# AlexandreRouma/SDRPlusPlus

Measured on NVIDIA H100. Metric: complex IQ MSamples/s through FFT + 8-VFO WFM chain, higher is better.
Workload: dtype f32

## Files before the change

### sdrplusplus_b200/csrc/engine.cpp

```cpp
#include "engine.h"
#include <chrono>
#include "../../include/b200dsp.h"
#include <cmath>
#include <cstdarg>
#include <cstdio>
#include <cstring>
#include <algorithm>
#include <map>
#include <functional>
#include <cstdlib>

namespace b200 {

static thread_local char g_err[512] = "";
void set_error(const char* fmt, ...) {
    va_list ap;
    va_start(ap, fmt);
    vsnprintf(g_err, sizeof(g_err), fmt, ap);
    va_end(ap);
}
const char* last_error() { return g_err; }
int cuda_fail(cudaError_t e, const char* what) {
    set_error("CUDA error %d (%s) in %s", (int)e, cudaGetErrorString(e), what);
    if (e == cudaErrorNoDevice || e == cudaErrorInsufficientDriver) { return B200_ENODEV; }
    return B200_ECUDA;
}

struct TraceRec { const char* label; cudaEvent_t ev; };
static std::vector<TraceRec> g_trace;
static int g_trace_on = -1;
bool trace_on() {
    if (g_trace_on < 0) { const char* e = getenv("B200_TRACE"); g_trace_on = (e && *e && *e != '0') ? 1 : 0; }
    return g_trace_on == 1;
}
void trace_mark(const char* label, cudaStream_t s) {
// ... 112 lines not shown
    }
    taps_dirty = false;
    return 0;
}

int XdStage::plan(int n) {
    n_in = n;
    chunk_offset = offset;
    chunk_phase0 = phase;
    chunk_retuned = retuned && n > 0;
    chunk_w_prev = w_prev;
    if (n > 0) { retuned = false; }
    n_out = (offset < n) ? (n - offset + D - 1) / D : 0;
    offset = offset + n_out * D - n;
    phase += w * (unsigned long long)(long long)n;
    return n_out;
}

int FirCStage::configure(const std::vector<float>& t, int decim_) {
    ntaps = (int)t.size();
    decim = decim_;
    hist = ntaps - 1;
    htaps = t;
    int rc = taps.alloc((size_t)ntaps * sizeof(float));
    if (rc) { return rc; }
    B200_CK(cudaMemcpy(taps.p, t.data(), (size_t)ntaps * sizeof(float), cudaMemcpyHostToDevice));
    return upload_pm(t, decim, 1);
}
int FirCStage::plan(int n) {
    n_in = n;
    chunk_offset = offset;
    n_out = (offset < n) ? (n - offset + decim - 1) / decim : 0;
    offset = offset + n_out * decim - n;
    return n_out;
}

int PolyStage::configure(int interp_, int decim_, const std::vector<float>& t) {
    interp = interp_;
    decim = decim_;
    std::vector<float> b = build_polyphase_bank(interp, t, tpp);
    hist = tpp - 1;
    int rc = bank.alloc(b.size() * sizeof(float));
    if (rc) { return rc; }
    B200_CK(cudaMemcpy(bank.p, b.data(), b.size() * sizeof(float), cudaMemcpyHostToDevice));
    {
        std::vector<float> kl(((size_t)tpp * interp + 3) & ~(size_t)3, 0.0f);
        for (int ph = 0; ph < interp; ph++) {
            for (int k = 0; k < tpp; k++) { kl[(size_t)k * interp + ph] = b[(size_t)ph * tpp + k]; }
        }
        if ((rc = bank_kl.alloc(kl.size() * sizeof(float)))) { return rc; }
        B200_CK(cudaMemcpy(bank_kl.p, kl.data(), kl.size() * sizeof(float), cudaMemcpyHostToDevice));
    }
    return upload_pm(b, decim, interp);
}
int PolyStage::plan(int n) {
    n_in = n;
    chunk_phase = phase;
    chunk_offset = offset;
    long long avail = ((long long)n - offset) * interp - phase;
    long long no = avail > 0 ? (avail + decim - 1) / decim : 0;
    n_out = (int)no;
    long long tend = (long long)phase + no * decim;
    offset = (int)((long long)offset + tend / interp - n);
    phase = (int)(tend % interp);
    return n_out;
}
// ... 87 lines not shown
    B200_CK(cudaMemcpy(state.p, init_state, sizeof(init_state), cudaMemcpyHostToDevice));
    return 0;
}

int SeqStage::configure_noise_blanker(double rate, double level) {
    memset(&proto, 0, sizeof(proto));
    proto.kind = 3;
    proto.nb_rate = (float)rate;
    proto.nb_inv_rate = 1.0f - proto.nb_rate;
    proto.nb_level = (float)level;
    in_es = 2;
    out_es = 2;
    memset(init_state, 0, sizeof(init_state));
    init_state[7] = 1.0f;
    int rc = state.alloc(sizeof(init_state));
    if (rc) { return rc; }
    B200_CK(cudaMemcpy(state.p, init_state, sizeof(init_state), cudaMemcpyHostToDevice));
    return 0;
}
int FmIfStage::configure(int nbins) {
    if (!fmif_supported(nbins)) { set_error("FM IF noise reduction: %d bins (supported: 2 ... %d)", nbins, 64); return B200_EINVAL; }
    bins = nbins;
    hist = bins - 1;
    const std::vector<float> w = fmif_window(bins), t = dft_twiddles(bins);
    int rc;
    if ((rc = win.alloc(w.size() * sizeof(float), false)) || (rc = tw.alloc(t.size() * sizeof(float), false))) { return rc; }
    B200_CK(cudaMemcpy(win.p, w.data(), w.size() * sizeof(float), cudaMemcpyHostToDevice));
    B200_CK(cudaMemcpy(tw.p, t.data(), t.size() * sizeof(float), cudaMemcpyHostToDevice));
    return 0;
}

int Chain::finalize(int max_in, bool dbl_first, const FuseCfg* fuse) {
    if (st.empty()) { set_error("empty chain"); return B200_EINVAL; }
    int cap = max_in;
    if (dbl_first && st.size() >= 2 && st[0]->kind == K_XD) { st[1]->dbl = true; }
    for (auto& s : st) {
        if (s->kind != K_XD) {
            int rc = s->alloc_in(cap);
            if (rc) { return rc; }
        }
        else { s->cap_in = cap; }
        cap = s->max_out(cap);
    }
    {
        int c2 = max_in;
        for (auto& s : st) {
            if (s->kind == K_STEREO) {
                StereoStage* q = (StereoStage*)s.get();
                int rc2;
                if ((rc2 = q->p.alloc(((size_t)c2 + 8) * sizeof(float2), false)) || (rc2 = q->vco.alloc(((size_t)c2 + 8) * sizeof(float2), false))) { return rc2; }
            }
            c2 = s->max_out(c2);
        }
    }
    out_es = st.back()->out_es;
    out_cap = cap;
    int rc = out.alloc(((size_t)cap + 8) * out_es * sizeof(float));
    if (rc) { return rc; }
    if (fuse) { fcfg = *fuse; }
    rc = plan_fused();
    if (rc) { return rc; }
    B200_CK(cudaDeviceSynchronize());
    return 0;
}

static bool ft_fusable(const Stage* s) {
    switch (s->kind) {
    case K_FIRC: return s->in_es == 2;
    case K_POLY: return s->in_es == 2 && ((const PolyStage*)s)->interp <= 64;
    case K_QUAD: case K_FIRR: case K_M2S: return true;
    default: return false;
    }
}
static void ft_describe(const Stage* s, FtStage& d) {
    memset(&d, 0, sizeof(d));
    d.D = 1; d.L = 1; d.T = 1;
    d.hist = s->hist;
    d.es = s->in_es;
    switch (s->kind) {
    case K_FIRC: { const FirCStage* f = (const FirCStage*)s; d.kind = FT_FIRC; d.T = f->ntaps; d.D = f->decim; break; }
    case K_POLY: { const PolyStage* f = (const PolyStage*)s; d.kind = FT_POLY; d.T = f->tpp; d.D = f->decim; d.L = f->interp; break; }
    case K_QUAD: { const QuadStage* f = (const QuadStage*)s; d.kind = FT_QUAD; d.scale = f->inv_dev; break; }
    case K_FIRR: { const FirRStage* f = (const FirRStage*)s; d.kind = FT_FIRR; d.T = f->ntaps; d.dup = f->stereo; break; }
    default: d.kind = FT_M2S; d.dup = 1; break;
    }
    d.taps = s->taps_pm.as<float>();
    d.ntap_f = s->pm_floats;
}
static long long ft_need_len(const FtStage& d, long long len) {
    switch (d.kind) {
    case FT_FIRC: case FT_FIRR: return (len - 1) * d.D + d.T;
    case FT_POLY: return ((len - 1) * d.D + d.L - 1) / d.L + d.T + 1;
    case FT_QUAD: return len + 1;
// ... 363 lines not shown
        t.ev.push_back(a);
        t.ev.push_back(b);
    }
    cudaEvent_t t0 = t.ev[t.used], t1 = t.ev[t.used + 1];
    t.used += 2;
    cudaEventRecord(t0, s);
    return t1;
}
int Scheduler::group_stats(int group, double* ms_total, int* n) {
    if (group < 0 || group > 2) { set_error("bad timer group"); return B200_EINVAL; }
    Timer& t = timers[group];
    double tot = 0.0;
    for (size_t i = 0; i + 1 < t.used; i += 2) {
        B200_CK(cudaEventSynchronize(t.ev[i + 1]));
        float ms = 0.0f;
        B200_CK(cudaEventElapsedTime(&ms, t.ev[i], t.ev[i + 1]));
        tot += ms;
    }
    *ms_total = tot;
    *n = (int)(t.used / 2);
    t.used = 0;
    return 0;
}
int Scheduler::reset_raw() {
    if (raw_hist.p) { B200_CK(cudaMemset(raw_hist.p, 0, raw_hist.bytes)); B200_CK(cudaDeviceSynchronize()); }
    return 0;
}

static int apply_pending_taps(FirCStage* f, cudaStream_t s) {
    if (f->pending.empty()) { return 0; }
    (void)s;
    B200_CK(cudaDeviceSynchronize());
    const int newT = (int)f->pending.size(), oldT = f->ntaps;
    const int newH = newT - 1, oldH = oldT - 1;
    const size_t bytes = ((size_t)newH + f->cap_in + Scheduler::STAGE_SPARE) * f->in_es * sizeof(float);
    DevBuf nb, nb2;
    int rc = nb.alloc(bytes);
    if (rc) { return rc; }
    if (f->dbl && (rc = nb2.alloc(bytes))) { return rc; }
    int keep = std::min(newH, oldH);
    const float* live = f->dbl ? ((f->par ? f->inbuf.as<float>() : f->inbuf_alt.as<float>())) : f->inbuf.as<float>();
    float* live_new = f->dbl ? ((f->par ? nb.as<float>() : nb2.as<float>())) : nb.as<float>();
    if (keep > 0) {
        B200_CK(cudaMemcpy(live_new + (size_t)(newH - keep) * f->in_es, live + (size_t)(oldH - keep) * f->in_es,
                           (size_t)keep * f->in_es * sizeof(float), cudaMemcpyDeviceToDevice));
    }
    std::swap(f->inbuf.p, nb.p);
    std::swap(f->inbuf.bytes, nb.bytes);
    if (f->dbl) {
        std::swap(f->inbuf_alt.p, nb2.p);
        std::swap(f->inbuf_alt.bytes, nb2.bytes);
    }
    if (f->fmid) {
        DevBuf h0, h1;
        const size_t hb = ((size_t)newH + 8) * f->in_es * sizeof(float);
        if ((rc = h0.alloc(hb)) || (rc = h1.alloc(hb))) { return rc; }
        if (keep > 0) {
            B200_CK(cudaMemcpy(h0.as<float>() + (size_t)(newH - keep) * f->in_es, f->fh[f->fpar].as<float>() + (size_t)(oldH - keep) * f->in_es,
                               (size_t)keep * f->in_es * sizeof(float), cudaMemcpyDeviceToDevice));
        }
        std::swap(f->fh[f->fpar].p, h0.p); std::swap(f->fh[f->fpar].bytes, h0.bytes);
        std::swap(f->fh[f->fpar ^ 1].p, h1.p); std::swap(f->fh[f->fpar ^ 1].bytes, h1.bytes);
    }
    rc = f->taps.alloc((size_t)newT * sizeof(float));
    if (rc) { return rc; }
    B200_CK(cudaMemcpy(f->taps.p, f->pending.data(), (size_t)newT * sizeof(float), cudaMemcpyHostToDevice));
    if ((rc = f->upload_pm(f->pending, f->decim, 1))) { return rc; }
    f->htaps = f->pending;
    f->ntaps = newT;
    f->hist = newH;
    if (f->decim != 1) { f->offset = 0; }
    f->pending.clear();
    B200_CK(cudaDeviceSynchronize());
    return 0;
}

static thread_local LaunchRec* g_rec = nullptr;
struct RecScope {
    explicit RecScope(LaunchRec* r) { g_rec = r; }
    ~RecScope() { g_rec = nullptr; }
};
static inline int rec_tag(const FirParams&) { return LaunchRec::T_FIR; }
static inline int rec_tag(const PolyParams&) { return LaunchRec::T_POLY; }
static inline int rec_tag(const FirRParams&) { return LaunchRec::T_FIRR; }
static inline int rec_tag(const QuadParams&) { return LaunchRec::T_QUAD; }
static inline int rec_tag(const SeqParams&) { return LaunchRec::T_SEQ; }
static inline int rec_tag(const M2SParams&) { return LaunchRec::T_M2S; }
static inline int rec_tag(const ScaleParams&) { return LaunchRec::T_SCALE; }
static inline int rec_tag(const CarryParams&) { return LaunchRec::T_CARRY; }
static inline int rec_tag(const FmIfParams&) { return LaunchRec::T_FMIF; }
static inline int rec_tag(const RxlParams&) { return LaunchRec::T_RXL; }

void LaunchRec::add(int tag, void* fn, const void* p, size_t size, int a, int b, size_t c) {
    const size_t off = (bytes.size() + 15) & ~(size_t)15;
    bytes.resize(off + size, 0);
    memcpy(bytes.data() + off, p, size);
    items.push_back(Item{ tag, fn, off, size, a, b, c, cur_branch });
}
unsigned long long LaunchRec::hash() const {
    unsigned long long h = 0x9E3779B97F4A7C15ULL ^ (unsigned long long)items.size();
    auto mix = [&](unsigned long long v) { h ^= v; h *= 0xD6E8FEB86659FD93ULL; h ^= h >> 32; };
    for (const Item& it : items) {
        mix((unsigned long long)it.tag | ((unsigned long long)it.branch << 32)); mix((unsigned long long)(uintptr_t)it.fn); mix((unsigned long long)it.size);
        mix((unsigned long long)(unsigned)it.a | ((unsigned long long)(unsigned)it.b << 32)); mix((unsigned long long)it.c);
    }
    const size_t n8 = bytes.size() / 8;
    const unsigned char* b = bytes.data();
    for (size_t i = 0; i < n8; i++) { unsigned long long v; memcpy(&v, b + 8 * i, 8); mix(v); }
    for (size_t i = n8 * 8; i < bytes.size(); i++) { mix(b[i]); }
    return h;
}
int LaunchRec::replay(cudaStream_t s0, long long* nlaunch) const {
    bool two = false;
    for (const Item& it : items) { two = two || it.branch != 0; }
    if (two) {
        if (!aux || !ev_fork || !ev_join) { set_error("launch list: no second stream"); return B200_ESTATE; }
        B200_CK(cudaEventRecord(ev_fork, s0));
        B200_CK(cudaStreamWaitEvent(aux, ev_fork, 0));
    }
    for (const Item& it : items) {
        cudaStream_t s = it.branch ? aux : s0;
        const void* q = bytes.data() + it.off;
        cudaError_t e = cudaSuccess;
        int nl = 1;
        switch (it.tag) {
        case T_DFR: e = launch_dfir_reg(*(const DfrParams*)q, it.a, it.b, s); break;
        case T_FIR: e = ((cudaError_t (*)(const FirParams&, cudaStream_t))it.fn)(*(const FirParams*)q, s); break;
        case T_POLY: e = ((cudaError_t (*)(const PolyParams&, cudaStream_t))it.fn)(*(const PolyParams*)q, s); break;
        case T_FIRR: e = ((cudaError_t (*)(const FirRParams&, cudaStream_t))it.fn)(*(const FirRParams*)q, s); break;
        case T_QUAD: e = launch_quad(*(const QuadParams*)q, s); break;
        case T_SEQ: e = launch_seq(*(const SeqParams*)q, s); break;
        case T_M2S: e = launch_m2s(*(const M2SParams*)q, s); break;
        case T_SCALE: e = launch_scale(*(const ScaleParams*)q, s); break;
        case T_CARRY: e = launch_carry(*(const CarryParams*)q, s); break;
        case T_FMIF: e = launch_fmif(*(const FmIfParams*)q, s); break;
        case T_RXL: e = launch_rxl(*(const RxlParams*)q, s); break;
        case T_STEREO: nl = 0; e = launch_stereo(*(const StParams*)q, s, &nl); break;
        case T_SQUELCH: nl = 0; e = launch_squelch(*(const SqParams*)q, s, &nl); break;
        case T_FUSED: e = launch_tail_fused(*(const FtParams*)q, it.a, it.b, it.c, s); break;
        default: set_error("launch list: unknown tag %d", it.tag); return B200_EINVAL;
        }
        if (e != cudaSuccess) { return cuda_fail(e, "kernel launch (tail list)"); }
        if (nlaunch) { *nlaunch += nl; }
    }
    if (two) {
        B200_CK(cudaEventRecord(ev_join, aux));
        B200_CK(cudaStreamWaitEvent(s0, ev_join, 0));
    }
    return 0;
}
void Scheduler::drop_graphs() {
    for (auto& kv : graphs) { if (kv.second.exec) { cudaGraphExecDestroy(kv.second.exec); } }
    graphs.clear();
}

template <class P, class L>
static int flush_batch(P& p, L launch, cudaStream_t s, long long& launches) {
    if (p.njobs == 0) { return 0; }
    if (g_rec) {
        g_rec->add(rec_tag(p), (void*)launch, &p, sizeof(P));
        p.njobs = 0;
        return 0;
    }
    cudaError_t e = launch(p, s);
    if (e != cudaSuccess) { return cuda_fail(e, "kernel launch"); }
    launches++;
    p.njobs = 0;
    return 0;
}
// ... 387 lines not shown
                    if (sg->kind == K_FIRC) { d.off = ((FirCStage*)sg)->chunk_offset; }
                    if (sg->kind == K_POLY) { d.off = ((PolyStage*)sg)->chunk_offset; d.phase = ((PolyStage*)sg)->chunk_phase; }
                    if (i > 0) {
                        d.hist_rd = sg->fh[sg->fpar].as<float>();
                        d.hist_wr = sg->fh[sg->fpar ^ 1].as<float>();
                        sg->fpar ^= 1;
                    }
                }
                J.src = c->st[c->fp.beg]->base();
                J.out = c->st[c->fp.end - 1]->out_ptr;
                J.slabs = std::max(1, (J.st[nst - 1].n_out + ob - 1) / ob);
                max_slabs = std::max(max_slabs, J.slabs);
                if (fpar.njobs == B200_BATCH) { int rc = flush(); if (rc) { return rc; } }
            }
            int rc = flush();
            if (rc) { return rc; }
        }
    }
    for (size_t lvl = 0; lvl < depth; lvl++) {
        FirParams fp; zero_params(fp, use_rec);
        FirParams fpr; zero_params(fpr, use_rec);
        PolyParams pp; zero_params(pp, use_rec);
        PolyParams ppr; zero_params(ppr, use_rec);
        FirRParams rpr; zero_params(rpr, use_rec);
        QuadParams qp; zero_params(qp, use_rec);
        FirRParams rp; zero_params(rp, use_rec);
        SeqParams sp; zero_params(sp, use_rec);
        M2SParams mp; zero_params(mp, use_rec);
        ScaleParams cp2; zero_params(cp2, use_rec);
        StParams stp; zero_params(stp, use_rec);
        SqParams sqp; zero_params(sqp, use_rec);
        FmIfParams fmp; zero_params(fmp, use_rec);
        RxlParams xlp; zero_params(xlp, use_rec);
        auto sq_flush = [&]() -> int {
            if (sqp.njobs == 0) { return 0; }
            int nl = 0;
            if (g_rec) { g_rec->add(LaunchRec::T_SQUELCH, nullptr, &sqp, sizeof(sqp)); }
            else {
                cudaError_t e = launch_squelch(sqp, ts, &nl);
                if (e != cudaSuccess) { return cuda_fail(e, "launch_squelch"); }
            }
            launches += nl;
            sqp.njobs = 0; sqp.max_n = 0;
            return 0;
        };
        auto st_flush = [&]() -> int {
            if (stp.njobs == 0) { return 0; }
            int nl = 0;
            if (g_rec) { g_rec->add(LaunchRec::T_STEREO, nullptr, &stp, sizeof(stp)); }
            else {
                cudaError_t e = launch_stereo(stp, ts, &nl);
                if (e != cudaSuccess) { return cuda_fail(e, "launch_stereo"); }
            }
            launches += nl;
            stp.njobs = 0; stp.max_n = 0;
            return 0;
        };
        for (Chain* c : chains) {
            if (lvl >= c->st.size()) { continue; }
            if (c->fp.active && lvl >= 1 && (int)lvl < c->fp.end) { continue; }
            Stage* s = c->st[lvl].get();
            int rc = 0;
            switch (s->kind) {
            case K_XD: break;
            case K_FIRC: {
                FirCStage* f = (FirCStage*)s;
                if (f->n_out <= 0) { break; }
                if (dfr_ok(f)) { rc = dfr_push(f); break; }
                if (fuse.pre_reg > 0 && f->decim == 1 && f->in_es == 2 && f->ntaps <= 2000 && f->chunk_offset == 0) {
                    FirJob& jr = fpr.job[fpr.njobs++];
                    jr.in = (const float2*)f->base(); jr.out = (float2*)f->out_ptr; jr.taps = f->taps.as<float>();
                    jr.ntaps = f->ntaps; jr.decim = 1; jr.offset = 0; jr.n_out = f->n_out;
                    fpr.max_out = std::max(fpr.max_out, f->n_out);
                    if (fpr.njobs == B200_BATCH) { rc = flush_batch(fpr, launch_fir_reg, ts, launches); fpr.max_out = 0; }
                    break;
                }
                FirJob& j = fp.job[fp.njobs++];
                j.in = (const float2*)f->base(); j.out = (float2*)f->out_ptr; j.taps = f->taps.as<float>();
                j.ntaps = f->ntaps; j.decim = f->decim; j.offset = f->chunk_offset; j.n_out = f->n_out;
                fp.max_out = std::max(fp.max_out, f->n_out);
                if (fp.njobs == B200_BATCH) { rc = flush_batch(fp, launch_fir_c, ts, launches); fp.max_out = 0; }
                break;
            }
            case K_POLY: {
                PolyStage* f = (PolyStage*)s;
                if (f->n_out <= 0) { break; }
                const bool regp = fuse.pre_reg > 0 && f->in_es == 2 && f->tpp <= 512 && poly_reg_supported(f->interp, f->decim);
                if (regp && ppr.njobs > 0 && (ppr.job[0].interp != f->interp || ppr.job[0].decim != f->decim)) {
                    rc = flush_batch(ppr, launch_poly_reg, ts, launches); ppr.max_out = 0;
                    if (rc) { break; }
                }
                PolyJob& j = regp ? ppr.job[ppr.njobs++] : pp.job[pp.njobs++];
                j.in = (const float2*)f->base(); j.out = (float2*)f->out_ptr; j.bank = f->bank.as<float>();
                j.tpp = f->tpp; j.interp = f->interp; j.decim = f->decim; j.phase0 = f->chunk_phase; j.offset0 = f->chunk_offset;
                j.n_out = f->n_out;
// ... 81 lines not shown
                }
                FmIfJob& j = fmp.job[fmp.njobs++];
                j.in = (const float2*)f->base(); j.out = (float2*)f->out_ptr; j.win = f->win.as<float>(); j.tw = f->tw.as<float2>();
                j.n = f->n_out; j.bins = f->bins;
                fmp.max_n = std::max(fmp.max_n, f->n_out);
                if (fmp.njobs == B200_BATCH) { rc = flush_batch(fmp, launch_fmif, ts, launches); fmp.max_n = 0; }
                break;
            }
            case K_SQUELCH: {
                SquelchStage* f = (SquelchStage*)s;
                if (f->n_out <= 0) { break; }
                SqJob& j = sqp.job[sqp.njobs++];
                j.in = (const float2*)f->in_data(); j.out = (float2*)f->out_ptr; j.partial = f->partial.as<float>(); j.n = f->n_out; j.level = f->level;
                sqp.max_n = std::max(sqp.max_n, f->n_out);
                if (sqp.njobs == B200_BATCH) { rc = sq_flush(); }
                break;
            }
            case K_M2S: {
                if (s->n_out <= 0) { break; }
                M2SJob& j = mp.job[mp.njobs++];
                j.in = s->in_data(); j.out = s->out_ptr; j.n = s->n_out;
                mp.max_n = std::max(mp.max_n, s->n_out);
                if (mp.njobs == B200_BATCH) { rc = flush_batch(mp, launch_m2s, ts, launches); mp.max_n = 0; }
                break;
            }
            }
            if (rc) { return rc; }
        }
        int rc;
        if ((rc = dfr_flush())) { return rc; }
        if ((rc = flush_batch(fpr, launch_fir_reg, ts, launches))) { return rc; }
        if ((rc = flush_batch(ppr, launch_poly_reg, ts, launches))) { return rc; }
        if ((rc = flush_batch(rpr, launch_firr_reg, ts, launches))) { return rc; }
        if ((rc = flush_batch(fp, launch_fir_c, ts, launches))) { return rc; }
        if ((rc = flush_batch(pp, launch_poly, ts, launches))) { return rc; }
        if ((rc = flush_batch(qp, launch_quad, ts, launches))) { return rc; }
        if ((rc = flush_batch(rp, launch_fir_r, ts, launches))) { return rc; }
        if ((rc = flush_batch(sp, launch_seq, ts, launches))) { return rc; }
        if ((rc = flush_batch(mp, launch_m2s, ts, launches))) { return rc; }
        if ((rc = flush_batch(cp2, launch_scale, ts, launches))) { return rc; }
        if ((rc = flush_batch(fmp, launch_fmif, ts, launches))) { return rc; }
        if ((rc = flush_batch(xlp, launch_rxl, ts, launches))) { return rc; }
        if ((rc = st_flush())) { return rc; }
        if ((rc = sq_flush())) { return rc; }
    }
    CarryParams cp;
    zero_params(cp, use_rec);
    auto push = [&](const CarryJob& j) -> int {
        cp.job[cp.njobs++] = j;
        if (cp.njobs == CARRY_BATCH) { return flush_batch(cp, launch_carry, ts, launches); }
        return 0;
    };
    for (Chain* c : chains) {
        for (auto& sp : c->st) {
            Stage* s = sp.get();
            if (s->kind == K_XD || s->hist <= 0 || s->fmid) { continue; }
            if (s->n_in <= 0 && !s->dbl) { continue; }
            CarryJob j;
            memset(&j, 0, sizeof(j));
            j.dst = s->other_base(); j.a = s->base(); j.b = s->in_data();
            j.h = s->hist; j.la = s->hist; j.lb = s->n_in; j.esize = s->in_es; j.bfmt = -1; j.scale = 0.0f;
            int rc = push(j);
            if (rc) { return rc; }
        }
    }
    int rcf = flush_batch(cp, launch_carry, ts, launches);
    if (rcf) { return rcf; }
    return 0;
    };
    if (nsplit == 1) {
        rec.cur_branch = 0;
        int rcs = tail_section(all_chains);
        if (rcs) { return rcs; }
    }
    else {
        const size_t half = (all_chains.size() + 1) / 2;
        std::vector<Chain*> ga(all_chains.begin(), all_chains.begin() + half), gb(all_chains.begin() + half, all_chains.end());
        rec.cur_branch = 0;
        int rcs = tail_section(ga);
        if (rcs) { return rcs; }
        rec.cur_branch = 1;
        if ((rcs = tail_section(gb))) { return rcs; }
        rec.cur_branch = 0;
    }
    if (use_rec) {
        g_rec = nullptr;
        int rcg = launch_recorded(ts, graph_tails > 0 || (graph_tails < 0 && count <= graph_max_count));
        if (rcg) { return rcg; }
    }
// ... 10 lines not shown
```

### sdrplusplus_b200/csrc/engine.h

```cpp
#pragma once
#include <cuda_runtime.h>
#include <cstdint>
#include <memory>
#include <mutex>
#include <string>
#include <vector>
#include <unordered_map>
#include "kernels.cuh"
#include "design.h"

namespace b200 {

void trace_mark(const char* label, cudaStream_t s);
void trace_dump(const char* title);
bool trace_on();

void set_error(const char* fmt, ...);
const char* last_error();
int cuda_fail(cudaError_t e, const char* what);
#define B200_CK(call)                                                     \
    do {                                                                  \
        cudaError_t _e = (call);                                          \
        if (_e != cudaSuccess) { return b200::cuda_fail(_e, #call); }     \
    } while (0)
// ... 5 lines not shown
    DevBuf(const DevBuf&) = delete;
    DevBuf& operator=(const DevBuf&) = delete;
    ~DevBuf() { release(); }
    int alloc(size_t n, bool zero = true);
    void release();
    template <class T> T* as() const { return (T*)p; }
};

enum StageKind { K_XD, K_FIRC, K_POLY, K_QUAD, K_FIRR, K_SEQ, K_M2S, K_SCALE, K_STEREO, K_SQUELCH, K_FMIF, K_RXL };

struct Stage {
    StageKind kind;
    int in_es = 2, out_es = 2;
    int hist = 0;
    int cap_in = 0;
    DevBuf inbuf;
    DevBuf inbuf_alt;
    bool dbl = false;
    int par = 0;
    int n_in = 0, n_out = 0;
    float* out_ptr = nullptr;
    DevBuf fh[2];
    int fpar = 0;
    bool fmid = false;
    DevBuf taps_pm;
    int pm_floats = 0;
    int upload_pm(const std::vector<float>& t, int rows_per_set, int sets);
    virtual ~Stage() {}
    virtual int plan(int n) = 0;
    virtual int max_out(int n) const = 0;
    virtual void reset_state() {}
    float* base() const { return (dbl && par) ? inbuf_alt.as<float>() : inbuf.as<float>(); }
    float* other_base() const { return (dbl && !par) ? inbuf_alt.as<float>() : inbuf.as<float>(); }
    float* in_data() const { return base() + (size_t)hist * in_es; }
    int alloc_in(int cap);
};

struct XdStage : Stage {
    int D = 1, T = 1;
    std::vector<float> h;
    double offset_rad = 0.0;
    unsigned long long phase = 0, w = 0, w_prev = 0;
    bool retuned = false, chunk_retuned = false; unsigned long long chunk_w_prev = 0;
    DevBuf hdev;
    int offset = 0;
    DevBuf gpad;
    int gpad_len = 0;
    int QP = 1;
    bool taps_dirty = true;
    XdStage() { kind = K_XD; }
    void configure(int D_, const std::vector<float>& taps);
    void set_offset_rad(double rad);
    int upload_taps(cudaStream_t s);
    int plan(int n) override;
    int max_out(int n) const override { return (n + D - 1) / D + 1; }
    void reset_state() override { phase = 0; offset = 0; retuned = false; }
    unsigned long long chunk_phase0 = 0; int chunk_offset = 0;
};

struct FirCStage : Stage {
    int ntaps = 1, decim = 1, offset = 0, chunk_offset = 0;
    DevBuf taps;
    std::vector<float> htaps;
    std::vector<float> pending;
    FirCStage() { kind = K_FIRC; }
    int configure(const std::vector<float>& t, int decim_);
    int plan(int n) override;
    int max_out(int n) const override { return (n + decim - 1) / decim + 1; }
    void reset_state() override { offset = 0; }
};

struct PolyStage : Stage {
    int interp = 1, decim = 1, tpp = 1, phase = 0, offset = 0, chunk_phase = 0, chunk_offset = 0;
    DevBuf bank, bank_kl;
    PolyStage() { kind = K_POLY; }
    int configure(int interp_, int decim_, const std::vector<float>& taps);
    int plan(int n) override;
    int max_out(int n) const override { return (int)(((long long)n * interp + decim - 1) / decim) + 2; }
    void reset_state() override { phase = 0; offset = 0; }
};

struct QuadStage : Stage {
    float inv_dev = 1.0f;
    QuadStage() { kind = K_QUAD; out_es = 1; hist = 1; }
    int configure(double deviationHz, double samplerate);
    int plan(int n) override { n_in = n; n_out = n; return n; }
    int max_out(int n) const override { return n; }
};

struct FirRStage : Stage {
    int ntaps = 1, stereo = 0;
    DevBuf taps;
    FirRStage() { kind = K_FIRR; in_es = 1; out_es = 1; }
    int configure(const std::vector<float>& t, bool stereo_);
    int plan(int n) override { n_in = n; n_out = n; return n; }
    int max_out(int n) const override { return n; }
};

struct SeqStage : Stage {
    SeqJob proto;
    DevBuf state;
    float init_state[SEQ_STATE_FLOATS];
// ... 47 lines not shown
    unsigned long long w = 0, phase = 0, chunk_phase0 = 0;
    RxlStage() { kind = K_RXL; in_es = 1; out_es = 2; }
    void set_offset_rad(double rad);
    int plan(int n) override { n_in = n; n_out = n; chunk_phase0 = phase; phase += w * (unsigned long long)(long long)n; return n; }
    int max_out(int n) const override { return n; }
    void reset_state() override { phase = 0; }
};

struct FmIfStage : Stage {
    int bins = 32;
    DevBuf win, tw;
    FmIfStage() { kind = K_FMIF; in_es = 2; out_es = 2; }
    int configure(int nbins);
    int plan(int n) override { n_in = n; n_out = n; return n; }
    int max_out(int n) const override { return n; }
};

struct ScaleStage : Stage {
    float gain = 1.0f;
    ScaleStage(int es, float g) { kind = K_SCALE; in_es = es; out_es = es; gain = g; }
    int plan(int n) override { n_in = n; n_out = n; return n; }
    int max_out(int n) const override { return n; }
};

struct Chain {
    std::vector<std::unique_ptr<Stage>> st;
    DevBuf out;
    int out_es = 2;
    int out_cap = 0;
    int n_out = 0;
    float* out_override = nullptr;
    bool raw_input() const { return !st.empty() && st[0]->kind == K_XD; }
    int chan_fir = -1;
    FusedPlan fp;
    FuseCfg fcfg;
    int plan_fused();
    int finalize(int max_in, bool dbl_first = false, const FuseCfg* fuse = nullptr);
    int plan(int n);
    int max_out(int n) const;
    int peek(int n) const;
    void reset_state();
    int add_rxvfo(double inSR, double outSR, double bw, double offset);
    int add_xlator(double offsetHz, double samplerate);
    int add_power_decim(int ratio);
    int add_resampler(double inSR, double outSR);
    int add_fir_c(const std::vector<float>& taps, int decim);
    int add_fir_r(const std::vector<float>& taps, bool stereo);
    int add_quad(double deviationHz, double samplerate);
    int add_wfm(double deviationHz, double samplerate, bool lowPass, bool stereo = false);
    int add_nfm(double samplerate, double bandwidth, bool lowPass);
    int add_am(int agcMode, double bandwidth, double attack, double decay, double dcRate, double samplerate);
    int add_ssb(int mode, double bandwidth, double samplerate, double attack, double decay);
    int add_deemph(double tau, double samplerate);
    int add_af_chain(double afSamplerate, double audioSamplerate, bool highPass, double deemphTau);
    int add_wfm_rds(double deviationHz, double samplerate);
    int add_noise_blanker(double rate, double level);
    int add_fmif(int bins);
    int add_squelch(double level);
    int add_volume(double volume, bool muted);
};

struct LaunchRec {
    enum Tag { T_DFR = 1, T_FIR, T_POLY, T_FIRR, T_QUAD, T_SEQ, T_M2S, T_SCALE, T_STEREO, T_SQUELCH, T_FUSED, T_CARRY, T_FMIF, T_RXL };
    struct Item { int tag; void* fn; size_t off, size; int a, b; size_t c; int branch; };
    int cur_branch = 0;
    cudaStream_t aux = nullptr;
    cudaEvent_t ev_fork = nullptr, ev_join = nullptr;
    std::vector<Item> items;
    std::vector<unsigned char> bytes;
    void clear() { items.clear(); bytes.clear(); }
    void add(int tag, void* fn, const void* p, size_t size, int a = 0, int b = 0, size_t c = 0);
    unsigned long long hash() const;
    int replay(cudaStream_t s, long long* nlaunch) const;
};

struct Scheduler {
    cudaStream_t stream = nullptr;
    cudaStream_t tail_stream = nullptr;
    cudaEvent_t ev_stage1[2] = { nullptr, nullptr }, ev_tail[2] = { nullptr, nullptr };
    unsigned long long chunk_idx = 0;
    cudaStream_t out_stream() const { return tail_stream ? tail_stream : stream; }
    int enable_overlap(cudaStream_t tail);
    long long launches = 0;
    int graph_tails = -1;
    int graph_max_count = 1 << 30;
    int tail_split = 1;
    cudaStream_t tail_stream2 = nullptr;
    struct GraphEntry { cudaGraphExec_t exec = nullptr; long long launches = 0; std::vector<unsigned char> key; };
    std::unordered_map<unsigned long long, GraphEntry> graphs;
    LaunchRec rec;
    long long graph_hits = 0, graph_misses = 0;
    void drop_graphs();
    int launch_recorded(cudaStream_t ts, bool may_graph);
    long long host_ns[4] = { 0, 0, 0, 0 };
    int s1_variant = 8;
    FuseCfg fuse;
// ... 22 lines not shown
```

### sdrplusplus_b200/csrc/kernels.cuh

```cuda
#pragma once
#include <cuda_runtime.h>
#include <stdint.h>

#define B200_BATCH 16

enum { FMT_CF32 = 0, FMT_CS16 = 1, FMT_CS8 = 2 };

struct XdJob {
    float2* out;
    const float2* gpad;
    unsigned long long phase0;
    unsigned long long w;
    int offset;
    int n_out;
    int T;
    const float* h;
    unsigned long long w_prev;
    int retuned;
};
struct XdParams {
    const void* in;
    const float2* hist;
    int hist_len;
    int count;
// ... 26 lines not shown
    FirJob job[B200_BATCH];
};

bool dfir_reg_supported(int D, int T);
cudaError_t launch_dfir_reg(const DfrParams& p, int D, int T, cudaStream_t s);

struct PolyJob {
    const float2* in;
    float2* out;
    const float* bank;
    int tpp, interp, decim, phase0, offset0, n_out;
    const float* bank_kl;
    long long in_len;
};
struct PolyParams { int njobs; int max_out; PolyJob job[B200_BATCH]; };
bool poly_reg_supported(int interp, int decim);
cudaError_t launch_poly_reg(const PolyParams& p, cudaStream_t s);

struct QuadJob {
    const float2* in;
    float* out;
    float inv_dev;
    int n;
};
struct QuadParams { int njobs; int max_n; QuadJob job[B200_BATCH]; };

struct FirRJob {
    const float* in;
    float* out;
    const float* taps;
    int ntaps, n_out, stereo;
};
struct FirRParams { int njobs; int max_out; FirRJob job[B200_BATCH]; };

#define FT_MAXST 8
#define FT_R 9
enum { FT_FIRC = 0, FT_POLY = 1, FT_QUAD = 2, FT_FIRR = 3, FT_M2S = 4 };
struct FtStage {
    int kind;
    int T;
    int D;
    int L;
    int off;
    int phase;
    int n_in, n_out;
    int hist;
    int es;
    int buf;
    int pitch;
    int tap_off, qpitch;
    int ntap_f;
    int dup;
    float scale;
    const float* taps;
    const float* hist_rd;
    float* hist_wr;
};
struct FtJob {
    int nst, slabs, OB, OT0;
    int stg2, pad;
    int s0_direct, stg3;
    int nat_off, stg_floats;
    const float* taps_nat;
    const float* src;
    float* out;
    FtStage st[FT_MAXST];
// ... 216 lines not shown
```

### sdrplusplus_b200/csrc/tails_reg.cuh

```cuda
#pragma once

#define TR_THREADS 128

template <int L, int M>
struct PolyGeom {
    static constexpr int W = ((L - 1) * M) / L + 1;
    __host__ __device__ static constexpr int off(int i) { return (i * M) / L; }
    __host__ __device__ static constexpr int ph(int i) { return (i * M) % L; }
};

#define PR_SPLIT 4
#define PR_PER 32
template <int L, int M>
__global__ void __launch_bounds__(TR_THREADS) k_poly_reg(const __grid_constant__ PolyParams p) {
    using G = PolyGeom<L, M>;
    extern __shared__ __align__(16) float2 tr_sm[];
    const PolyJob& J = p.job[blockIdx.y];
    pdl_trigger();
    const int tpp = J.tpp;
    int m_a = 0;
    while (((J.phase0 + m_a * M) % L) != 0) { m_a++; }
    const int g0 = blockIdx.x * PR_PER;
    const long long mfirst = (long long)m_a - L + (long long)g0 * L;
    if (mfirst >= J.n_out) { return; }
// ... 278 lines not shown
            frr_block(acc, ea, eb, oa, ob, eg + (kb + 1) * 3, og + (kb + 1) * 3, tq + kb * 8);
            frr_block(acc, eb, ea, ob, oa, eg + (kb + 2) * 3, og + (kb + 2) * 3, tq + kb * 8 + 8);
        }
        if (kb < n) { frr_block(acc, ea, eb, oa, ob, eg + (kb + 1) * 3, og + (kb + 1) * 3, tq + kb * 8); }
    }
#pragma unroll
    for (int i = 0; i < 8; i++) { red[(q * 32 + lane) * 9 + i] = acc[i].x + acc[i].y; }
    __syncthreads();
#pragma unroll
    for (int h = 0; h < TS_TILE / TR_THREADS; h++) {
        const int o = threadIdx.x + h * TR_THREADS;
        if (mt + o < J.n_out) {
            const int idx = (o >> 3) * 9 + (o & 7);
            const float v = (red[idx] + red[32 * 9 + idx]) + (red[2 * 32 * 9 + idx] + red[3 * 32 * 9 + idx]);
            if (J.stereo) { reinterpret_cast<float2*>(J.out)[mt + o] = make_float2(v, v); }
            else { J.out[mt + o] = v; }
        }
    }
}
cudaError_t launch_firr_reg(const FirRParams& p, cudaStream_t s) {
    if (p.njobs <= 0 || p.max_out <= 0) { return cudaSuccess; }
    int maxT = 0;
    for (int v = 0; v < p.njobs; v++) { maxT = p.job[v].ntaps > maxT ? p.job[v].ntaps : maxT; }
    const int Tp = (maxT + 7) & ~7;
    const int npairs = (TS_TILE + Tp + 8) / 2 + 4;
    const int ngroups = (npairs + 3) / 4 + 1;
    const size_t smem = ((size_t)(Tp + 8) / 2 + (size_t)ngroups * 3 * 2 * 2 + (size_t)TS_SPLIT * 32 * 9 / 2 + 8) * sizeof(float2);
    if ((int)smem > kernels_max_smem_optin()) { return cudaErrorInvalidValue; }
    cudaError_t e = set_smem(k_firr_reg, smem);
    if (e != cudaSuccess) { return e; }
    dim3 grid((unsigned)((p.max_out + TS_TILE - 1) / TS_TILE), (unsigned)p.njobs);
    return launch_chain(k_firr_reg, grid, dim3(TR_THREADS), smem, s, p);
}
```

Measured before the change: 84650.

## Fuse complex FIR, quadrature demod and audio FIR into one kernel

Adds a fused kernel that runs the channel complex FIR, the FM quadrature demodulator and the real audio FIR in a single launch. Intermediates stay in shared memory, and the FIR history is extended so the audio FIR's lookback can be recomputed from raw input. The aim is to remove two launches and the global-memory round trips for the intermediate buffers. The cost is redundant recomputation of overlap samples per block, plus extra bookkeeping for tap-change transitions that uses the previous taps. The fused path is used only when the generic fused-tail plan is inactive and pre_reg is enabled.

```diff
diff --git a/sdrplusplus_b200/csrc/engine.cpp b/sdrplusplus_b200/csrc/engine.cpp
--- a/sdrplusplus_b200/csrc/engine.cpp
+++ b/sdrplusplus_b200/csrc/engine.cpp
@@ -1,6 +1,7 @@
 #include "engine.h"
 #include <chrono>
 #include "../../include/b200dsp.h"
+#include <climits>
 #include <cmath>
 #include <cstdarg>
 #include <cstdio>
@@ -179,6 +180,11 @@
     chunk_offset = offset;
     n_out = (offset < n) ? (n - offset + decim - 1) / decim : 0;
     offset = offset + n_out * decim - n;
+    chunk_trans = trans; chunk_hpos = hpos; chunk_zpos = zpos;
+    if (trans) {
+        hpos -= n; zpos -= n;
+        if (hpos <= -tail_taps && zpos <= -(tail_taps + ntaps - 1)) { trans = false; }
+    }
     return n_out;
 }
 
@@ -332,12 +338,27 @@
 
 int Chain::finalize(int max_in, bool dbl_first, const FuseCfg* fuse) {
     if (st.empty()) { set_error("empty chain"); return B200_EINVAL; }
+    if (fuse) { fcfg = *fuse; }
+    int rc = plan_fused();
+    if (rc) { return rc; }
+    fqf = -1;
+    for (size_t i = 0; !fp.active && fcfg.pre_reg > 0 && i + 2 < st.size() && fqf < 0; i++) {
+        const Stage* a = st[i].get();
+        if (a->kind == K_FIRC && a->in_es == 2 && ((const FirCStage*)a)->decim == 1 && ((const FirCStage*)a)->ntaps <= 2000 &&
+            st[i + 1]->kind == K_QUAD && st[i + 2]->kind == K_FIRR && ((const FirRStage*)st[i + 2].get())->ntaps <= 2000) {
+            fqf = (int)i;
+            FirCStage* f = (FirCStage*)st[i].get();
+            f->tail_taps = ((const FirRStage*)st[i + 2].get())->ntaps;
+            f->hist = std::max(f->hist, f->ntaps - 1 + f->tail_taps);
+        }
+    }
     int cap = max_in;
     if (dbl_first && st.size() >= 2 && st[0]->kind == K_XD) { st[1]->dbl = true; }
-    for (auto& s : st) {
-        if (s->kind != K_XD) {
-            int rc = s->alloc_in(cap);
-            if (rc) { return rc; }
+    for (size_t i = 0; i < st.size(); i++) {
+        Stage* s = st[i].get();
+        if (s->kind != K_XD && !(fqf >= 0 && (i == (size_t)fqf + 1 || i == (size_t)fqf + 2))) {
+            int rc2 = s->alloc_in(cap);
+            if (rc2) { return rc2; }
         }
         else { s->cap_in = cap; }
         cap = s->max_out(cap);
@@ -355,10 +376,7 @@
     }
     out_es = st.back()->out_es;
     out_cap = cap;
-    int rc = out.alloc(((size_t)cap + 8) * out_es * sizeof(float));
-    if (rc) { return rc; }
-    if (fuse) { fcfg = *fuse; }
-    rc = plan_fused();
+    rc = out.alloc(((size_t)cap + 8) * out_es * sizeof(float));
     if (rc) { return rc; }
     B200_CK(cudaDeviceSynchronize());
     return 0;
@@ -788,13 +806,13 @@
     (void)s;
     B200_CK(cudaDeviceSynchronize());
     const int newT = (int)f->pending.size(), oldT = f->ntaps;
-    const int newH = newT - 1, oldH = oldT - 1;
+    const int oldH = f->hist, newH = f->tail_taps > 0 ? std::max(oldH, newT - 1 + f->tail_taps) : newT - 1;
     const size_t bytes = ((size_t)newH + f->cap_in + Scheduler::STAGE_SPARE) * f->in_es * sizeof(float);
     DevBuf nb, nb2;
     int rc = nb.alloc(bytes);
     if (rc) { return rc; }
     if (f->dbl && (rc = nb2.alloc(bytes))) { return rc; }
-    int keep = std::min(newH, oldH);
+    int keep = f->tail_taps > 0 ? oldH : std::min(newH, oldH);
     const float* live = f->dbl ? ((f->par ? f->inbuf.as<float>() : f->inbuf_alt.as<float>())) : f->inbuf.as<float>();
     float* live_new = f->dbl ? ((f->par ? nb.as<float>() : nb2.as<float>())) : nb.as<float>();
     if (keep > 0) {
@@ -817,6 +835,14 @@
         }
         std::swap(f->fh[f->fpar].p, h0.p); std::swap(f->fh[f->fpar].bytes, h0.bytes);
         std::swap(f->fh[f->fpar ^ 1].p, h1.p); std::swap(f->fh[f->fpar ^ 1].bytes, h1.bytes);
+    }
+    if (f->tail_taps > 0) {
+        std::swap(f->taps_prev.p, f->taps.p);
+        std::swap(f->taps_prev.bytes, f->taps.bytes);
+        f->ntaps_prev = oldT;
+        f->hpos = 0;
+        f->zpos = -std::min(oldT - 1, newT - 1);
+        f->trans = true;
     }
     rc = f->taps.alloc((size_t)newT * sizeof(float));
     if (rc) { return rc; }
@@ -846,6 +872,7 @@
 static inline int rec_tag(const CarryParams&) { return LaunchRec::T_CARRY; }
 static inline int rec_tag(const FmIfParams&) { return LaunchRec::T_FMIF; }
 static inline int rec_tag(const RxlParams&) { return LaunchRec::T_RXL; }
+static inline int rec_tag(const FqfParams&) { return LaunchRec::T_FQF; }
 
 void LaunchRec::add(int tag, void* fn, const void* p, size_t size, int a, int b, size_t c) {
     const size_t off = (bytes.size() + 15) & ~(size_t)15;
@@ -891,6 +918,7 @@
         case T_CARRY: e = launch_carry(*(const CarryParams*)q, s); break;
         case T_FMIF: e = launch_fmif(*(const FmIfParams*)q, s); break;
         case T_RXL: e = launch_rxl(*(const RxlParams*)q, s); break;
+        case T_FQF: e = launch_fqf_reg(*(const FqfParams*)q, s); break;
         case T_STEREO: nl = 0; e = launch_stereo(*(const StParams*)q, s, &nl); break;
         case T_SQUELCH: nl = 0; e = launch_squelch(*(const SqParams*)q, s, &nl); break;
         case T_FUSED: e = launch_tail_fused(*(const FtParams*)q, it.a, it.b, it.c, s); break;
@@ -1344,6 +1372,7 @@
         SqParams sqp; zero_params(sqp, use_rec);
         FmIfParams fmp; zero_params(fmp, use_rec);
         RxlParams xlp; zero_params(xlp, use_rec);
+        FqfParams fqp; zero_params(fqp, use_rec);
         auto sq_flush = [&]() -> int {
             if (sqp.njobs == 0) { return 0; }
             int nl = 0;
@@ -1371,8 +1400,27 @@
         for (Chain* c : chains) {
             if (lvl >= c->st.size()) { continue; }
             if (c->fp.active && lvl >= 1 && (int)lvl < c->fp.end) { continue; }
+            if (c->fqf >= 0 && (lvl == (size_t)c->fqf + 1 || lvl == (size_t)c->fqf + 2)) { continue; }
             Stage* s = c->st[lvl].get();
             int rc = 0;
+            if ((int)lvl == c->fqf) {
+                FirCStage* f = (FirCStage*)s;
+                const QuadStage* qs = (const QuadStage*)c->st[lvl + 1].get();
+                const FirRStage* r = (const FirRStage*)c->st[lvl + 2].get();
+                if (f->n_out <= 0) { continue; }
+                FqfJob& j = fqp.job[fqp.njobs++];
+                j.x = (const float2*)f->in_data(); j.out = r->out_ptr;
+                j.taps = f->taps.as<float>(); j.T = f->ntaps;
+                j.taps_h = f->chunk_trans ? f->taps_prev.as<float>() : j.taps; j.T_h = f->chunk_trans ? f->ntaps_prev : f->ntaps;
+                j.taps_af = r->taps.as<float>(); j.T_af = r->ntaps;
+                j.n = f->n_out; j.hist = f->hist;
+                j.hpos = f->chunk_trans ? f->chunk_hpos : INT_MIN / 2; j.zpos = f->chunk_trans ? f->chunk_zpos : INT_MIN / 2;
+                j.stereo = r->stereo; j.inv_dev = qs->inv_dev;
+                fqp.max_out = std::max(fqp.max_out, f->n_out);
+                if (fqp.njobs == B200_BATCH) { rc = flush_batch(fqp, launch_fqf_reg, ts, launches); fqp.max_out = 0; }
+                if (rc) { return rc; }
+                continue;
+            }
             switch (s->kind) {
             case K_XD: break;
             case K_FIRC: {
@@ -1520,6 +1568,7 @@
         if ((rc = flush_batch(fpr, launch_fir_reg, ts, launches))) { return rc; }
         if ((rc = flush_batch(ppr, launch_poly_reg, ts, launches))) { return rc; }
         if ((rc = flush_batch(rpr, launch_firr_reg, ts, launches))) { return rc; }
+        if ((rc = flush_batch(fqp, launch_fqf_reg, ts, launches))) { return rc; }
         if ((rc = flush_batch(fp, launch_fir_c, ts, launches))) { return rc; }
         if ((rc = flush_batch(pp, launch_poly, ts, launches))) { return rc; }
         if ((rc = flush_batch(qp, launch_quad, ts, launches))) { return rc; }
@@ -1540,9 +1589,10 @@
         return 0;
     };
     for (Chain* c : chains) {
-        for (auto& sp : c->st) {
-            Stage* s = sp.get();
+        for (size_t i = 0; i < c->st.size(); i++) {
+            Stage* s = c->st[i].get();
             if (s->kind == K_XD || s->hist <= 0 || s->fmid) { continue; }
+            if (c->fqf >= 0 && (i == (size_t)c->fqf + 1 || i == (size_t)c->fqf + 2)) { continue; }
             if (s->n_in <= 0 && !s->dbl) { continue; }
             CarryJob j;
             memset(&j, 0, sizeof(j));
diff --git a/sdrplusplus_b200/csrc/engine.h b/sdrplusplus_b200/csrc/engine.h
--- a/sdrplusplus_b200/csrc/engine.h
+++ b/sdrplusplus_b200/csrc/engine.h
@@ -61,7 +61,7 @@
     virtual void reset_state() {}
     float* base() const { return (dbl && par) ? inbuf_alt.as<float>() : inbuf.as<float>(); }
     float* other_base() const { return (dbl && !par) ? inbuf_alt.as<float>() : inbuf.as<float>(); }
-    float* in_data() const { return base() + (size_t)hist * in_es; }
+    float* in_data() const { float* b = base(); return b ? b + (size_t)hist * in_es : nullptr; }
     int alloc_in(int cap);
 };
 
@@ -92,11 +92,16 @@
     DevBuf taps;
     std::vector<float> htaps;
     std::vector<float> pending;
+    int tail_taps = 0;
+    DevBuf taps_prev;
+    int ntaps_prev = 0;
+    bool trans = false, chunk_trans = false;
+    int hpos = 0, zpos = 0, chunk_hpos = 0, chunk_zpos = 0;
     FirCStage() { kind = K_FIRC; }
     int configure(const std::vector<float>& t, int decim_);
     int plan(int n) override;
     int max_out(int n) const override { return (n + decim - 1) / decim + 1; }
-    void reset_state() override { offset = 0; }
+    void reset_state() override { offset = 0; trans = false; }
 };
 
 struct PolyStage : Stage {
@@ -210,6 +215,7 @@
     float* out_override = nullptr;
     bool raw_input() const { return !st.empty() && st[0]->kind == K_XD; }
     int chan_fir = -1;
+    int fqf = -1;
     FusedPlan fp;
     FuseCfg fcfg;
     int plan_fused();
@@ -239,7 +245,7 @@
 };
 
 struct LaunchRec {
-    enum Tag { T_DFR = 1, T_FIR, T_POLY, T_FIRR, T_QUAD, T_SEQ, T_M2S, T_SCALE, T_STEREO, T_SQUELCH, T_FUSED, T_CARRY, T_FMIF, T_RXL };
+    enum Tag { T_DFR = 1, T_FIR, T_POLY, T_FIRR, T_QUAD, T_SEQ, T_M2S, T_SCALE, T_STEREO, T_SQUELCH, T_FUSED, T_CARRY, T_FMIF, T_RXL, T_FQF };
     struct Item { int tag; void* fn; size_t off, size; int a, b; size_t c; int branch; };
     int cur_branch = 0;
     cudaStream_t aux = nullptr;
diff --git a/sdrplusplus_b200/csrc/kernels.cuh b/sdrplusplus_b200/csrc/kernels.cuh
--- a/sdrplusplus_b200/csrc/kernels.cuh
+++ b/sdrplusplus_b200/csrc/kernels.cuh
@@ -82,6 +82,18 @@
     int ntaps, n_out, stereo;
 };
 struct FirRParams { int njobs; int max_out; FirRJob job[B200_BATCH]; };
+
+struct FqfJob {
+    const float2* x;
+    float* out;
+    const float* taps;
+    const float* taps_h;
+    const float* taps_af;
+    int T, T_h, T_af, n, hist, hpos, zpos, stereo;
+    float inv_dev;
+};
+struct FqfParams { int njobs; int max_out; FqfJob job[B200_BATCH]; };
+cudaError_t launch_fqf_reg(const FqfParams& p, cudaStream_t s);
 
 #define FT_MAXST 8
 #define FT_R 9
diff --git a/sdrplusplus_b200/csrc/tails_reg.cuh b/sdrplusplus_b200/csrc/tails_reg.cuh
--- a/sdrplusplus_b200/csrc/tails_reg.cuh
+++ b/sdrplusplus_b200/csrc/tails_reg.cuh
@@ -334,3 +334,208 @@
     dim3 grid((unsigned)((p.max_out + TS_TILE - 1) / TS_TILE), (unsigned)p.njobs);
     return launch_chain(k_firr_reg, grid, dim3(TR_THREADS), smem, s, p);
 }
+
+#define FQ_OB 384
+#define FQ_RA 3
+#define FQ_RC 3
+static_assert(FQ_OB == FQ_RA * TR_THREADS, "one audio output block per thread");
+__device__ __forceinline__ void fq_range(int T, int q, int& k0, int& k1) {
+    const int nb = (T + 7) >> 3, nbq = (nb + TS_SPLIT - 1) / TS_SPLIT;
+    k0 = 8 * q * nbq;
+    k1 = min(T, 8 * min(nb, (q + 1) * nbq));
+}
+template <bool ZERO>
+__device__ __forceinline__ void fq_chan(float2 (&c)[FQ_RC], const float2* xw0, const float* h0, int T, int zi0) {
+    float2 s01[FQ_RC], p2[FQ_RC];
+#pragma unroll
+    for (int q = 0; q < TS_SPLIT; q++) {
+        int k0, k1;
+        fq_range(T, q, k0, k1);
+        const float2* xw = xw0 + k0;
+        const float* h = h0 + k0;
+        const int n = k1 - k0, zi = zi0 - k0;
+        auto ld = [&](int s) { return (ZERO && s < zi) ? make_float2(0.0f, 0.0f) : xw[s]; };
+        float2 acc[FQ_RC], win[FQ_RC];
+#pragma unroll
+        for (int i = 0; i < FQ_RC; i++) { acc[i] = make_float2(0.0f, 0.0f); win[i] = ld(i); }
+        int k = 0;
+        for (; k + 2 * FQ_RC <= n; k += 2 * FQ_RC) {
+#pragma unroll
+            for (int kk = 0; kk < 2 * FQ_RC; kk += 2) {
+                const float2 h2 = *reinterpret_cast<const float2*>(h + k + kk);
+#pragma unroll
+                for (int i = 0; i < FQ_RC; i++) { acc[i] = ffma2(make_float2(h2.x, h2.x), win[(i + kk) % FQ_RC], acc[i]); }
+                win[kk % FQ_RC] = ld(k + kk + FQ_RC);
+#pragma unroll
+                for (int i = 0; i < FQ_RC; i++) { acc[i] = ffma2(make_float2(h2.y, h2.y), win[(i + kk + 1) % FQ_RC], acc[i]); }
+                win[(kk + 1) % FQ_RC] = ld(k + kk + 1 + FQ_RC);
+            }
+        }
+#pragma unroll
+        for (int kk = 0; kk < 2 * FQ_RC; kk++) {
+            if (k + kk < n) {
+                const float hk = h[k + kk];
+#pragma unroll
+                for (int i = 0; i < FQ_RC; i++) { acc[i] = ffma2(make_float2(hk, hk), win[(i + kk) % FQ_RC], acc[i]); }
+                win[kk % FQ_RC] = ld(k + kk + FQ_RC);
+            }
+        }
+#pragma unroll
+        for (int i = 0; i < FQ_RC; i++) {
+            if (q == 0) { s01[i] = acc[i]; }
+            else if (q == 1) { s01[i] = make_float2(s01[i].x + acc[i].x, s01[i].y + acc[i].y); }
+            else if (q == 2) { p2[i] = acc[i]; }
+            else { c[i] = make_float2(s01[i].x + (p2[i].x + acc[i].x), s01[i].y + (p2[i].y + acc[i].y)); }
+        }
+    }
+}
+__device__ __forceinline__ void fq_audio_part(float (&r)[FQ_RA], const float* dw, const float* h, int n) {
+    float ae[FQ_RA], ao[FQ_RA], win[FQ_RA];
+#pragma unroll
+    for (int i = 0; i < FQ_RA; i++) { ae[i] = 0.0f; ao[i] = 0.0f; win[i] = dw[i]; }
+    int k = 0;
+    for (; k + 2 * FQ_RA <= n; k += 2 * FQ_RA) {
+#pragma unroll
+        for (int kk = 0; kk < 2 * FQ_RA; kk += 2) {
+            const float2 h2 = *reinterpret_cast<const float2*>(h + k + kk);
+#pragma unroll
+            for (int i = 0; i < FQ_RA; i++) { ae[i] = __fmaf_rn(h2.x, win[(i + kk) % FQ_RA], ae[i]); }
+            win[kk % FQ_RA] = dw[k + kk + FQ_RA];
+#pragma unroll
+            for (int i = 0; i < FQ_RA; i++) { ao[i] = __fmaf_rn(h2.y, win[(i + kk + 1) % FQ_RA], ao[i]); }
+            win[(kk + 1) % FQ_RA] = dw[k + kk + 1 + FQ_RA];
+        }
+    }
+#pragma unroll
+    for (int kk = 0; kk < 2 * FQ_RA; kk++) {
+        if (k + kk < n) {
+            const float hk = h[k + kk];
+#pragma unroll
+            for (int i = 0; i < FQ_RA; i++) {
+                const float v = win[(i + kk) % FQ_RA];
+                if (kk & 1) { ao[i] = __fmaf_rn(hk, v, ao[i]); } else { ae[i] = __fmaf_rn(hk, v, ae[i]); }
+            }
+            win[kk % FQ_RA] = dw[k + kk + FQ_RA];
+        }
+    }
+#pragma unroll
+    for (int i = 0; i < FQ_RA; i++) { r[i] = ae[i] + ao[i]; }
+}
+__host__ __device__ inline int fq_ncr(int Ta) {
+    const int per = FQ_RC * TR_THREADS;
+    return (FQ_OB + Ta + per - 1) / per * per;
+}
+__host__ __device__ inline int fq_nx(int Ta, int Tm) { return (fq_ncr(Ta) + Tm + FQ_RC + 2) & ~1; }
+__host__ __device__ inline int fq_r4(int x) { return (x + 3) & ~3; }
+__global__ void __launch_bounds__(TR_THREADS) k_fqf_reg(const __grid_constant__ FqfParams p) {
+    extern __shared__ __align__(16) float2 tr_sm[];
+    const FqfJob& J = p.job[blockIdx.y];
+    pdl_trigger();
+    const int mt = blockIdx.x * FQ_OB;
+    if (mt >= J.n) { return; }
+    const int T = J.T, Th = J.T_h, Ta = J.T_af;
+    const bool two = J.taps_h != J.taps;
+    const int Tm = two ? max(T, Th) : T;
+    float* hc = reinterpret_cast<float*>(tr_sm);
+    float* hh = two ? hc + fq_r4(T) : hc;
+    float* ha = hc + fq_r4(T) + (two ? fq_r4(Th) : 0);
+    float* ang = ha + fq_r4(Ta);
+    float2* X = reinterpret_cast<float2*>(ang + fq_r4(FQ_OB + Ta));
+    const int nx = fq_nx(Ta, Tm);
+    for (int k = threadIdx.x; k < T; k += TR_THREADS) { hc[k] = __ldg(J.taps + k); }
+    if (two) { for (int k = threadIdx.x; k < Th; k += TR_THREADS) { hh[k] = __ldg(J.taps_h + k); } }
+    for (int k = threadIdx.x; k < Ta; k += TR_THREADS) { ha[k] = __ldg(J.taps_af + k); }
+    const int nout = min(FQ_OB, J.n - mt);
+    const int cb = mt - Ta;
+    const int nc = nout + Ta;
+    const int xlo = cb - (Tm - 1);
+    const int o = xlo - ((J.hist + xlo) & 1);
+    {
+        const int hi = mt + nout;
+        const float4* __restrict__ src = reinterpret_cast<const float4*>(J.x + o);
+        float4* X4 = reinterpret_cast<float4*>(X);
+        pdl_wait();
+        for (int i = threadIdx.x; i < nx / 2; i += TR_THREADS) {
+            const int s = o + 2 * i;
+            float4 v = make_float4(0.f, 0.f, 0.f, 0.f);
+            if (s < hi) {
+                v = __ldcg(src + i);
+                if (s + 1 >= hi) { v.z = 0.0f; v.w = 0.0f; }
+            }
+            X4[i] = v;
+        }
+    }
+    __syncthreads();
+    for (int r0 = threadIdx.x * FQ_RC; r0 < nc; r0 += FQ_RC * TR_THREADS) {
+        const int j0 = cb + r0;
+        float2 c[FQ_RC];
+        if (j0 < J.hpos) {
+            fq_chan<false>(c, X + (j0 - (Th - 1) - o), hh, Th, 0);
+#pragma unroll
+            for (int i = 0; i < FQ_RC; i++) { if (j0 + i < J.hpos && r0 + i < nc) { ang[r0 + i] = atan2f(c[i].y, c[i].x); } }
+        }
+        if (j0 + FQ_RC > J.hpos) {
+            const int xs = j0 - (T - 1);
+            if (J.zpos > xs) { fq_chan<true>(c, X + (xs - o), hc, T, J.zpos - xs); }
+            else { fq_chan<false>(c, X + (xs - o), hc, T, 0); }
+#pragma unroll
+            for (int i = 0; i < FQ_RC; i++) { if (j0 + i >= J.hpos && r0 + i < nc) { ang[r0 + i] = atan2f(c[i].y, c[i].x); } }
+        }
+    }
+    __syncthreads();
+    float* D = reinterpret_cast<float*>(X);
+    for (int r = threadIdx.x; r < FQ_OB + Ta + 2 * FQ_RA; r += TR_THREADS) {
+        float v = 0.0f;
+        if (r < nc - 1) {
+            float diff = __fsub_rn(ang[r + 1], ang[r]);
+            if (diff > FL_M_PI_REF) { diff = __fsub_rn(diff, 2.0f * FL_M_PI_REF); }
+            else if (diff <= -FL_M_PI_REF) { diff = __fadd_rn(diff, 2.0f * FL_M_PI_REF); }
+            v = __fmul_rn(diff, J.inv_dev);
+        }
+        D[r] = v;
+    }
+    __syncthreads();
+    const int m0 = threadIdx.x * FQ_RA;
+    if (m0 >= nout) { return; }
+    float s01[FQ_RA], v[FQ_RA];
+#pragma unroll
+    for (int q = 0; q < TS_SPLIT; q++) {
+        int k0, k1;
+        fq_range(Ta, q, k0, k1);
+        float r[FQ_RA];
+        fq_audio_part(r, D + m0 + k0, ha + k0, k1 - k0);
+#pragma unroll
+        for (int i = 0; i < FQ_RA; i++) {
+            if (q == 0) { s01[i] = r[i]; }
+            else if (q == 1) { s01[i] = s01[i] + r[i]; }
+            else if (q == 2) { v[i] = r[i]; }
+            else { v[i] = s01[i] + (v[i] + r[i]); }
+        }
+    }
+#pragma unroll
+    for (int i = 0; i < FQ_RA; i++) {
+        const int m = mt + m0 + i;
+        if (m0 + i < nout) {
+            if (J.stereo) { reinterpret_cast<float2*>(J.out)[m] = make_float2(v[i], v[i]); }
+            else { J.out[m] = v[i]; }
+        }
+    }
+}
+cudaError_t launch_fqf_reg(const FqfParams& p, cudaStream_t s) {
+    if (p.njobs <= 0 || p.max_out <= 0) { return cudaSuccess; }
+    int maxT = 0, maxTh = 0, maxTa = 0, maxTm = 0;
+    for (int v = 0; v < p.njobs; v++) {
+        const FqfJob& J = p.job[v];
+        const bool two = J.taps_h != J.taps;
+        maxT = std::max(maxT, J.T);
+        maxTh = std::max(maxTh, two ? J.T_h : 0);
+        maxTa = std::max(maxTa, J.T_af);
+        maxTm = std::max(maxTm, two ? std::max(J.T, J.T_h) : J.T);
+    }
+    const size_t smem = (size_t)(fq_r4(maxT) + fq_r4(maxTh) + fq_r4(maxTa) + fq_r4(FQ_OB + maxTa) + 2 * fq_nx(maxTa, maxTm)) * sizeof(float);
+    if ((int)smem > kernels_max_smem_optin()) { return cudaErrorInvalidValue; }
+    cudaError_t e = set_smem(k_fqf_reg, smem);
+    if (e != cudaSuccess) { return e; }
+    dim3 grid((unsigned)((p.max_out + FQ_OB - 1) / FQ_OB), (unsigned)p.njobs);
+    return launch_chain(k_fqf_reg, grid, dim3(TR_THREADS), smem, s, p);
+}
```

New measurement: 80450 (median of 6 runs). 5.0% lower.
